# mom-ocean/MOM6

Measured on AMD Instinct MI355X. Metric: simulated-days/wall-sec, higher is better.
Workload: dtype f64

## Files before the change

### mom6_amd/csrc/barotropic.hip

```cpp
#include <algorithm>
#include <type_traits>
#include <vector>
#include <cmath>
#include "mom6x_dev.h"


enum BTW {
  W_q = 0, W_DCor_u, W_DCor_v, W_gtot_E, W_gtot_W, W_gtot_N, W_gtot_S, W_eta, W_eta_PF,
  W_Cor_ref_u, W_Cor_ref_v, W_BT_force_u, W_BT_force_v, W_ubt, W_vbt, W_bt_rem_u, W_bt_rem_v,
  W_uhbt0, W_vhbt0, W_ubt_Cor, W_vbt_Cor, W_uhbt, W_vhbt, W_u_accel_bt, W_v_accel_bt,
  W_eta_src, W_e_anom, W_eta_sum, W_eta_wtd, W_ubt_wtd, W_vbt_wtd, W_eta_pred,
  W_uh0sum, W_vh0sum, W_ubt0, W_vbt0,
  W_f4u, W_f4u_2, W_f4u_3, W_f4u_4, W_f4v, W_f4v_2, W_f4v_3, W_f4v_4,
  W_BTCu,
  W_BTCv = W_BTCu + 10,
  W_BTtmp = W_BTCv + 10,
  W_uhn = W_BTtmp + 12,
  W_vhn,
  W_ubt2, W_vbt2, W_eta_pred2,
  W_COUNT
};

enum BTC { B_FA_EE = 0, B_FA_E0, B_FA_W0, B_FA_WW, B_uBT_WW, B_uBT_EE, B_crvW, B_crvE, B_uh_WW, B_uh_EE };

struct BTState {
  mom6x_barotropic_params P;
  double *frhatu, *frhatv, *IDatu, *IDatv, *ubtav, *vbtav, *eta_cor, *q_D, *D_u_Cor, *D_v_Cor;
  double *work;
  int nstep_last;
  unsigned long long *warn;
  double *warn_info;
  bool la_pending;
  const double *la_pbce;
  double la_underflow;
  bool fr_pending;
  const double *fr_hu, *fr_hv;
};

namespace {

__device__ __forceinline__ double *wp(double *work, const Dm &d, int m) { return work + (size_t)m * d.slab; }

__device__ __forceinline__ double find_uhbt(double u, const double *__restrict__ B, size_t c, size_t slab) {
  if (u == 0.0) return 0.0;
  const double uEE = B[B_uBT_EE * slab + c];
  if (u < uEE) return (u - uEE) * B[B_FA_EE * slab + c] + B[B_uh_EE * slab + c];
  if (u < 0.0) return u * (B[B_FA_E0 * slab + c] + B[B_crvE * slab + c] * (u * u));
  const double uWW = B[B_uBT_WW * slab + c];
  if (u <= uWW) return u * (B[B_FA_W0 * slab + c] + B[B_crvW * slab + c] * (u * u));
  return (u - uWW) * B[B_FA_WW * slab + c] + B[B_uh_WW * slab + c];
}

__global__ void k_bt_init_static(Dm d, const double *__restrict__ G, double Z_to_H, double Mean_SL,
                                 double cor_scale, double H_subroundoff, double *q_D, double *D_u_Cor,
                                 double *D_v_Cor, double *IDatu, double *IDatv) {
  const int i = -1 + blockIdx.x * blockDim.x + threadIdx.x;
  const int j = -1 + blockIdx.y * blockDim.y + threadIdx.y;
  if (i > d.ni - 1 || j > d.nj - 1) return;
  const int st = d.pitch;
  const size_t c = ix2(d, i, j);
  const double *bathyT = gm(G, d, MOM6X_G_bathyT), *areaT = gm(G, d, MOM6X_G_areaT), *mT = gm(G, d, MOM6X_G_mask2dT);
  const double *mCu = gm(G, d, MOM6X_G_mask2dCu), *mCv = gm(G, d, MOM6X_G_mask2dCv), *fBu = gm(G, d, MOM6X_G_CoriolisBu);
  if (j >= 0) {
    D_u_Cor[c] = 0.5 * (dmax(Mean_SL + bathyT[c + 1], 0.0) + dmax(Mean_SL + bathyT[c], 0.0)) * Z_to_H;
    if (mCu[c] > 0.) IDatu[c] = mCu[c] * 2.0 / (Z_to_H * ((bathyT[c + 1] + bathyT[c]) + 2.0 * Mean_SL));
    else IDatu[c] = 0.;
  }
  if (i >= 0) {
    D_v_Cor[c] = 0.5 * (dmax(Mean_SL + bathyT[c + st], 0.0) + dmax(Mean_SL + bathyT[c], 0.0)) * Z_to_H;
    if (mCv[c] > 0.) IDatv[c] = mCv[c] * 2.0 / (Z_to_H * ((bathyT[c + st] + bathyT[c]) + 2.0 * Mean_SL));
    else IDatv[c] = 0.;
  }
  if (mT[c] + mT[c + st] + mT[c + 1] + mT[c + 1 + st] > 0.) {
    q_D[c] = 0.25 * (cor_scale * fBu[c]) * ((areaT[c] + areaT[c + 1 + st]) + (areaT[c + 1] + areaT[c + st])) /
        (Z_to_H * dmax((((areaT[c] * dmax(Mean_SL + bathyT[c], 0.0)) +
                         (areaT[c + 1 + st] * dmax(Mean_SL + bathyT[c + 1 + st], 0.0))) +
                        ((areaT[c + 1] * dmax(Mean_SL + bathyT[c + 1], 0.0)) +
                         (areaT[c + st] * dmax(Mean_SL + bathyT[c + st], 0.0)))), H_subroundoff));
  } else {
    q_D[c] = 0.;
  }
}

// ... 243 lines not shown
    tmp[0 * slab + c] = -1.0e100; tmp[1 * slab + c] = 1.0e100;
    tmp[2 * slab + c] = Dat; tmp[3 * slab + c] = Dat; tmp[4 * slab + c] = Dat; tmp[5 * slab + c] = Dat;
  }
  if (i >= -1) {
    const double H2 = eta ? (bathyT[c + st] * Z_to_H + eta[c + st]) : ((bathyT[c + st] + Z_ref) * Z_to_H);
    double Dat = 0.0;
    if ((H1 > 0.0) && (H2 > 0.0)) Dat = gm(G, d, MOM6X_G_dx_Cv)[c] * (2.0 * H1 * H2) / (H1 + H2);
    tmp[6 * slab + c] = -1.0e100; tmp[7 * slab + c] = 1.0e100;
    tmp[8 * slab + c] = Dat; tmp[9 * slab + c] = Dat; tmp[10 * slab + c] = Dat; tmp[11 * slab + c] = Dat;
  }
}
__global__ void k_face_areas_eta(Dm d, const double *__restrict__ G, double Z_to_H, const double *__restrict__ eta, double *Bu, double *Bv,
                                 int isv, int iev, int jsv, int jev) {
  const int i = isv - 2 + blockIdx.x * blockDim.x + threadIdx.x;
  const int j = jsv - 2 + blockIdx.y * blockDim.y + threadIdx.y;
  if (i > iev + 1 || j > jev + 1) return;
  const int st = d.pitch;
  const size_t c = ix2(d, i, j), slab = (size_t)d.slab;
  const double *bathyT = gm(G, d, MOM6X_G_bathyT);
  const double H1 = bathyT[c] * Z_to_H + eta[c];
  if (j >= jsv - 1) {
    const double H2 = bathyT[c + 1] * Z_to_H + eta[c + 1];
    double Dat = 0.0;
    if ((H1 > 0.0) && (H2 > 0.0)) Dat = gm(G, d, MOM6X_G_dy_Cu)[c] * (2.0 * H1 * H2) / (H1 + H2);
    Bu[B_FA_EE * slab + c] = Dat; Bu[B_FA_E0 * slab + c] = Dat; Bu[B_FA_W0 * slab + c] = Dat; Bu[B_FA_WW * slab + c] = Dat;
  }
  if (i >= isv - 1) {
    const double H2 = bathyT[c + st] * Z_to_H + eta[c + st];
    double Dat = 0.0;
    if ((H1 > 0.0) && (H2 > 0.0)) Dat = gm(G, d, MOM6X_G_dx_Cv)[c] * (2.0 * H1 * H2) / (H1 + H2);
    Bv[B_FA_EE * slab + c] = Dat; Bv[B_FA_E0 * slab + c] = Dat; Bv[B_FA_W0 * slab + c] = Dat; Bv[B_FA_WW * slab + c] = Dat;
  }
}
__global__ void k_btcl(Dm d, const double *__restrict__ tmp, double *Bu, double *Bv, int hs) {
  const int i = -hs - 1 + blockIdx.x * blockDim.x + threadIdx.x;
  const int j = -hs - 1 + blockIdx.y * blockDim.y + threadIdx.y;
  if (i > d.ni - 1 + hs || j > d.nj - 1 + hs) return;
  const size_t c = ix2(d, i, j), slab = (size_t)d.slab;
  const double C1_3 = 1.0 / 3.0;
  for (int dir = 0; dir < 2; dir++) {
    if (dir == 0 && j < -hs) continue;
    if (dir == 1 && i < -hs) continue;
    const double *t = tmp + (size_t)(dir * 6) * slab;
    double *B = dir ? Bv : Bu;
    const double FA_EE = t[2 * slab + c], FA_E0 = t[3 * slab + c], FA_W0 = t[4 * slab + c], FA_WW = t[5 * slab + c];
    const double uBT_EE = 1.0 * t[0 * slab + c], uBT_WW = 1.0 * t[1 * slab + c];
    B[B_FA_EE * slab + c] = FA_EE; B[B_FA_E0 * slab + c] = FA_E0; B[B_FA_W0 * slab + c] = FA_W0; B[B_FA_WW * slab + c] = FA_WW;
    B[B_uBT_EE * slab + c] = uBT_EE; B[B_uBT_WW * slab + c] = uBT_WW;
    B[B_uh_EE * slab + c] = uBT_EE * (C1_3 * (2.0 * FA_E0 + FA_EE));
    B[B_uh_WW * slab + c] = uBT_WW * (C1_3 * (2.0 * FA_W0 + FA_WW));
    double crvW = 0.0, crvE = 0.0;
    if (fabs(uBT_WW) > 0.0) crvW = (C1_3 * (FA_WW - FA_W0)) / (uBT_WW * uBT_WW);
    if (fabs(uBT_EE) > 0.0) crvE = (C1_3 * (FA_EE - FA_E0)) / (uBT_EE * uBT_EE);
    B[B_crvW * slab + c] = crvW; B[B_crvE * slab + c] = crvE;
  }
}

__global__ void k_uhbt0(Dm d, const double *__restrict__ work_c, double *work) {
  const int i = -1 + blockIdx.x * blockDim.x + threadIdx.x;
  const int j = -1 + blockIdx.y * blockDim.y + threadIdx.y;
  if (i > d.ni - 1 || j > d.nj - 1) return;
  const size_t c = ix2(d, i, j), slab = (size_t)d.slab;
  if (j >= 0) work[W_uhbt0 * slab + c] = work_c[W_uh0sum * slab + c] - find_uhbt(work_c[W_ubt0 * slab + c], work_c + W_BTCu * slab, c, slab);
  if (i >= 0) work[W_vhbt0 * slab + c] = work_c[W_vh0sum * slab + c] - find_uhbt(work_c[W_vbt0 * slab + c], work_c + W_BTCv * slab, c, slab);
}

__global__ void k_find_Cor(Dm d, double *work, int Sadourny, int isvf, int ievf, int jsvf, int jevf) {
  const int i = isvf - 1 + blockIdx.x * blockDim.x + threadIdx.x;
  const int j = jsvf - 1 + blockIdx.y * blockDim.y + threadIdx.y;
  if (i > ievf + 1 || j > jevf + 1) return;
  const int st = d.pitch;
  const size_t c = ix2(d, i, j), slab = (size_t)d.slab;
  const double *q = work + W_q * slab, *DCor_u = work + W_DCor_u * slab, *DCor_v = work + W_DCor_v * slab;
  double *f4u = work + W_f4u * slab, *f4v = work + W_f4v * slab;
  if (j <= jevf) {
    if (Sadourny) {
      f4v[0 * slab + c] = 1.0 * DCor_u[c - 1] * q[c - 1];
      f4v[1 * slab + c] = 1.0 * DCor_u[c] * q[c];
      f4v[3 * slab + c] = 1.0 * DCor_u[c + st] * q[c];
      f4v[2 * slab + c] = 1.0 * DCor_u[c - 1 + st] * q[c - 1];
    } else {
      f4v[0 * slab + c] = 1.0 * DCor_u[c - 1] * ((q[c] + q[c - 1 - st]) + q[c - 1]) / 3.0;
      f4v[1 * slab + c] = 1.0 * DCor_u[c] * (q[c] + (q[c - 1] + q[c - st])) / 3.0;
      f4v[3 * slab + c] = 1.0 * DCor_u[c + st] * (q[c] + (q[c - 1] + q[c + st])) / 3.0;
      f4v[2 * slab + c] = 1.0 * DCor_u[c - 1 + st] * ((q[c] + q[c - 1 + st]) + q[c - 1]) / 3.0;
    }
  }
  if (i <= ievf) {
    if (Sadourny) {
      f4u[3 * slab + c] = 1.0 * DCor_v[c + 1] * q[c];
      f4u[2 * slab + c] = 1.0 * DCor_v[c] * q[c];
      f4u[0 * slab + c] = 1.0 * DCor_v[c - st] * q[c - st];
      f4u[1 * slab + c] = 1.0 * DCor_v[c + 1 - st] * q[c - st];
    } else {
      f4u[3 * slab + c] = 1.0 * DCor_v[c + 1] * (q[c] + (q[c + 1] + q[c - st])) / 3.0;
      f4u[2 * slab + c] = 1.0 * DCor_v[c] * (q[c] + (q[c - 1] + q[c - st])) / 3.0;
      f4u[0 * slab + c] = 1.0 * DCor_v[c - st] * ((q[c] + q[c - 1 - st]) + q[c - st]) / 3.0;
      f4u[1 * slab + c] = 1.0 * DCor_v[c + 1 - st] * ((q[c] + q[c + 1 - st]) + q[c - st]) / 3.0;
    }
  }
}

__global__ void k_cor_ref_eta_src(Dm d, const double *__restrict__ G, double *work, double *eta_cor, double Instep,
                                  int bound_BT_corr, double maxCFL_Idt, double dt, double Z_to_H, double Z_ref, double maxvel) {
  const int i = -1 + blockIdx.x * blockDim.x + threadIdx.x;
  const int j = -1 + blockIdx.y * blockDim.y + threadIdx.y;
  if (i > d.ni - 1 || j > d.nj - 1) return;
  const int st = d.pitch;
  const size_t c = ix2(d, i, j), slab = (size_t)d.slab;
  const double *f4u = work + W_f4u * slab, *f4v = work + W_f4v * slab;
  const double *ubt_Cor = work + W_ubt_Cor * slab, *vbt_Cor = work + W_vbt_Cor * slab;
  if (j >= 0)
    work[W_Cor_ref_u * slab + c] = (((f4u[3 * slab + c] * vbt_Cor[c + 1]) + (f4u[0 * slab + c] * vbt_Cor[c - st])) +
                                    ((f4u[2 * slab + c] * vbt_Cor[c]) + (f4u[1 * slab + c] * vbt_Cor[c + 1 - st])));
  if (i >= 0)
    work[W_Cor_ref_v * slab + c] = -1.0 * (((f4v[0 * slab + c] * ubt_Cor[c - 1]) + (f4v[3 * slab + c] * ubt_Cor[c + st])) +
                                           ((f4v[1 * slab + c] * ubt_Cor[c]) + (f4v[2 * slab + c] * ubt_Cor[c - 1 + st])));
  if (i >= 0 && j >= 0) {
    const double mT = gm(G, d, MOM6X_G_mask2dT)[c];
    double ec = eta_cor[c];
    if (bound_BT_corr == 2) {
      const double *bathyT = gm(G, d, MOM6X_G_bathyT), *dy_Cu = gm(G, d, MOM6X_G_dy_Cu), *dx_Cv = gm(G, d, MOM6X_G_dx_Cv);
      auto Dat = [&](size_t a, size_t bb, double len) {
        const double H1 = (bathyT[a] + Z_ref) * Z_to_H, H2 = (bathyT[bb] + Z_ref) * Z_to_H;
        double D = 0.0;
        if ((H1 > 0.0) && (H2 > 0.0)) D = len * (2.0 * H1 * H2) / (H1 + H2);
        return D;
      };
      const double DatuW = Dat(c - 1, c, dy_Cu[c - 1]), DatuE = Dat(c, c + 1, dy_Cu[c]);
      const double DatvN = Dat(c, c + st, dx_Cv[c]), DatvS = Dat(c - st, c, dx_Cv[c - st]);
      const double bound = dt * (gm(G, d, MOM6X_G_IareaT)[c] * 0.1 * maxvel * ((DatuW + DatuE) + (DatvN + DatvS)));
      if (fabs(ec) > bound) ec = copysign(bound, ec);
      eta_cor[c] = ec;
    } else if (bound_BT_corr && mT > 0.0) {
      if (ec > 0.0) {
        const double u_max_cor = gm(G, d, MOM6X_G_dxT)[c] * maxCFL_Idt, v_max_cor = gm(G, d, MOM6X_G_dyT)[c] * maxCFL_Idt;
        const double *Bu = work + W_BTCu * slab, *Bv = work + W_BTCv * slab;
        const double *uhbt0 = work + W_uhbt0 * slab, *vhbt0 = work + W_vhbt0 * slab;
        const double eta_cor_max = dt * (gm(G, d, MOM6X_G_IareaT)[c] *
            (((find_uhbt(u_max_cor, Bu, c, slab) + uhbt0[c]) - (find_uhbt(-u_max_cor, Bu, c - 1, slab) + uhbt0[c - 1])) +
             ((find_uhbt(v_max_cor, Bv, c, slab) + vhbt0[c]) - (find_uhbt(-v_max_cor, Bv, c - st, slab) + vhbt0[c - st]))));
        ec = dmin(ec, dmax(0.0, eta_cor_max));
      } else {
        const double Htot = gm(G, d, MOM6X_G_bathyT)[c] * Z_to_H + work[W_eta * slab + c];
        ec = dmax(ec, -dmax(0.0, Htot));
      }
      eta_cor[c] = ec;
    }
    work[W_eta_src * slab + c] = mT * (Instep * ec);
  }
// ... 24 lines not shown
__global__ void __launch_bounds__(256)
k_bt_pred(Dm d, const double *__restrict__ G, double *work, LoopArgs A, int p_ubt, int p_vbt, int p_pred, int sel) {
  const int i = I_BASE(A.isv - 1) + blockIdx.x * blockDim.x + threadIdx.x;
  const int j = A.jsv - 1 + blockIdx.y * blockDim.y + threadIdx.y;
  if (i < A.isv - 1 || i > A.iev + 1 || j > A.jev + 1) return;
  if (sel) { const bool own = (i >= 0 && i <= d.ni - 1 && j >= 0 && j <= d.nj - 1); if (own != (sel == 1)) return; }
  const int st = d.pitch;
  const size_t c = ix2(d, i, j), slab = (size_t)d.slab;
  double eta_PF_BT;
  if (A.project) {
    eta_PF_BT = work[W_eta * slab + c];
  } else {
    const double *ubt = work + (size_t)p_ubt * slab, *vbt = work + (size_t)p_vbt * slab;
    const double *Bu = work + W_BTCu * slab, *Bv = work + W_BTCv * slab;
    const double *uhbt0 = work + W_uhbt0 * slab, *vhbt0 = work + W_vhbt0 * slab;
    double uW, uE, vS, vN;
    if (A.have_uhn) {
      const double *uhn = work + W_uhn * slab, *vhn = work + W_vhn * slab;
      uW = uhn[c - 1]; uE = uhn[c]; vS = vhn[c - st]; vN = vhn[c];
    } else {
      uW = find_uhbt(ubt[c - 1], Bu, c - 1, slab) + uhbt0[c - 1];
      uE = find_uhbt(ubt[c], Bu, c, slab) + uhbt0[c];
      vS = find_uhbt(vbt[c - st], Bv, c - st, slab) + vhbt0[c - st];
      vN = find_uhbt(vbt[c], Bv, c, slab) + vhbt0[c];
    }
    eta_PF_BT = (work[W_eta * slab + c] + work[W_eta_src * slab + c]) +
                (A.dtbt * gm(G, d, MOM6X_G_IareaT)[c]) * ((uW - uE) + (vS - vN));
    work[(size_t)p_pred * slab + c] = eta_PF_BT;
  }
  if (A.find_etaav && (fabs(A.wt_accel2) > 0.0) && i >= 0 && i <= d.ni - 1 && j >= 0 && j <= d.nj - 1)
    work[W_eta_sum * slab + c] = work[W_eta_sum * slab + c] + A.wt_accel2 * eta_PF_BT;
}

__device__ __forceinline__ void f4u_of(const double *__restrict__ q, const double *__restrict__ DCor_v, size_t c, int st, int Sadourny,
                                       double &f0, double &f1, double &f2, double &f3) {
  if (Sadourny) {
    f3 = 1.0 * DCor_v[c + 1] * q[c];
    f2 = 1.0 * DCor_v[c] * q[c];
    f0 = 1.0 * DCor_v[c - st] * q[c - st];
    f1 = 1.0 * DCor_v[c + 1 - st] * q[c - st];
  } else {
    f3 = 1.0 * DCor_v[c + 1] * (q[c] + (q[c + 1] + q[c - st])) / 3.0;
    f2 = 1.0 * DCor_v[c] * (q[c] + (q[c - 1] + q[c - st])) / 3.0;
    f0 = 1.0 * DCor_v[c - st] * ((q[c] + q[c - 1 - st]) + q[c - st]) / 3.0;
    f1 = 1.0 * DCor_v[c + 1 - st] * ((q[c] + q[c + 1 - st]) + q[c - st]) / 3.0;
  }
}
__device__ __forceinline__ void f4v_of(const double *__restrict__ q, const double *__restrict__ DCor_u, size_t c, int st, int Sadourny,
                                       double &f0, double &f1, double &f2, double &f3) {
  if (Sadourny) {
    f0 = 1.0 * DCor_u[c - 1] * q[c - 1];
    f1 = 1.0 * DCor_u[c] * q[c];
    f3 = 1.0 * DCor_u[c + st] * q[c];
    f2 = 1.0 * DCor_u[c - 1 + st] * q[c - 1];
  } else {
    f0 = 1.0 * DCor_u[c - 1] * ((q[c] + q[c - 1 - st]) + q[c - 1]) / 3.0;
    f1 = 1.0 * DCor_u[c] * (q[c] + (q[c - 1] + q[c - st])) / 3.0;
    f3 = 1.0 * DCor_u[c + st] * (q[c] + (q[c - 1] + q[c + st])) / 3.0;
    f2 = 1.0 * DCor_u[c - 1 + st] * ((q[c] + q[c - 1 + st]) + q[c - 1]) / 3.0;
  }
}

template <int DIR>
__device__ __forceinline__ void bt_face_update(const Dm &d, const double *__restrict__ G, const double *work, const LoopArgs &A, size_t c, int st,
                                               size_t slab, const double *etaB, double vel, double n0, double n1, double n2, double n3,
                                               int bracket_bug, double &newv, double &CorPF) {
  const double *eta_PF = work + W_eta_PF * slab;
  double Cor, PF, f0, f1, f2, f3;
  if (DIR == 0) {
    const double *gE = work + W_gtot_E * slab, *gW = work + W_gtot_W * slab;
    PF = (((etaB[c] - eta_PF[c]) * gE[c]) - ((etaB[c + 1] - eta_PF[c + 1]) * gW[c + 1])) * A.dgeo_de * gm(G, d, MOM6X_G_IdxCu)[c];
    f4u_of(work + W_q * slab, work + W_DCor_v * slab, c, st, A.Sadourny, f0, f1, f2, f3);
    Cor = (((f3 * n0) + (f0 * n1)) + ((f2 * n2) + (f1 * n3))) - work[W_Cor_ref_u * slab + c];
    newv = work[W_bt_rem_u * slab + c] * (vel + A.dtbt * ((work[W_BT_force_u * slab + c] + Cor) + PF));
  } else {
    const double *gN = work + W_gtot_N * slab, *gS = work + W_gtot_S * slab;
    PF = (((etaB[c] - eta_PF[c]) * gN[c]) - ((etaB[c + st] - eta_PF[c + st]) * gS[c + st])) * A.dgeo_de * gm(G, d, MOM6X_G_IdyCv)[c];
    f4v_of(work + W_q * slab, work + W_DCor_u * slab, c, st, A.Sadourny, f0, f1, f2, f3);
    if (bracket_bug) Cor = -1.0 * (((f0 * n0) + (f1 * n1)) + ((f3 * n2) + (f2 * n3))) - work[W_Cor_ref_v * slab + c];
    else Cor = -1.0 * (((f0 * n0) + (f3 * n2)) + ((f1 * n1) + (f2 * n3))) - work[W_Cor_ref_v * slab + c];
    newv = work[W_bt_rem_v * slab + c] * (vel + A.dtbt * ((work[W_BT_force_v * slab + c] + Cor) + PF));
  }
  if (fabs(newv) < A.vel_underflow) newv = 0.0;
  CorPF = Cor + PF;
}

template <int DIR>
__global__ void __launch_bounds__(256)
k_bt_vel(Dm d, const double *__restrict__ G, double *work, double *btav, double *hbtav, LoopArgs A,
         int a0, int a1, int b0, int b1, int bracket_bug) {
  const int i = I_BASE(a0) + blockIdx.x * blockDim.x + threadIdx.x;
  const int j = b0 + blockIdx.y * blockDim.y + threadIdx.y;
  if (i < a0 || i > a1 || j > b1) return;
  const int st = d.pitch;
  const size_t c = ix2(d, i, j), slab = (size_t)d.slab;
// ... 530 lines not shown
  Au.Instep = Instep; Au.RZ_to_H = c->GV.RZ_to_H; Au.vel_underflow = P.vel_underflow; Au.nstep = nstep;
  Au.wt_uv_bug = P.wt_uv_bug; Au.visc_rem_u_uh0 = P.visc_rem_u_uh0; Au.strong_drag = P.strong_drag;
  ColArgs Av = Au;
  Av.visc_rem = visc_rem_v; Av.frhat = s->frhatv; Av.U_Cor = V_Cor; Av.uh0 = vh0; Av.u_uh0 = v_vh0; Av.U_in = V_in;
  Av.bc_accel = bc_accel_v; Av.tau = tauy; Av.tau_bot = tauy_bot; Av.IDat = s->IDatv;
  Av.ubt_Cor = work + W_vbt_Cor * slab; Av.gtot_m = work + W_gtot_N * slab; Av.gtot_p = work + W_gtot_S * slab;
  Av.uh0sum = work + W_vh0sum * slab; Av.ubt0 = work + W_vbt0 * slab; Av.ubt = work + W_vbt * slab;
  Av.BT_force = work + W_BT_force_v * slab; Av.bt_rem = work + W_bt_rem_v * slab;
  if (s->fr_pending) {
    Au.hf = s->fr_hu; Av.hf = s->fr_hv; Au.h_neglect = Av.h_neglect = c->GV.H_subroundoff;
    KLAUNCH(c, "k_bt_col<0>", (k_bt_col<0, true>), grid3(nxa(d.ni + 1, -1), d.nj, 1, b), b, d, c->G, Au);
    KLAUNCH(c, "k_bt_col<1>", (k_bt_col<1, true>), grid3(d.ni, d.nj + 1, 1, b), b, d, c->G, Av);
  } else {
    { const int rcm = bt_frhat_materialize(c); if (rcm) return rcm; }
    KLAUNCH(c, "k_bt_col<0>", (k_bt_col<0, false>), grid3(nxa(d.ni + 1, -1), d.nj, 1, b), b, d, c->G, Au);
    KLAUNCH(c, "k_bt_col<1>", (k_bt_col<1, false>), grid3(d.ni, d.nj + 1, 1, b), b, d, c->G, Av);
  }

  double *tmp = work + W_BTtmp * slab;
  if (BT_cont) KLAUNCH(c, "k_btcont_copy", k_btcont_copy, grid3(d.ni + 1, d.nj + 1, 1, b), b, d, *BT_cont, tmp);
  else KLAUNCH(c, "k_face_areas_as_fits", k_face_areas_as_fits, grid3(d.ni + 3, d.nj + 3, 1, b), b, d, c->G, P.Z_ref, c->GV.Z_to_H, tmp,
               P.nonlinear_continuity ? (const double *)(work + W_eta * slab) : (const double *)nullptr);
  {
    double *f[18]; int stg[18], nks[18];
    for (int m = 0; m < 12; m++) { f[m] = tmp + (size_t)m * slab; stg[m] = (m < 6) ? 1 : 2; nks[m] = 1; }
    double *g[] = { work + W_gtot_E * slab, work + W_gtot_N * slab, work + W_gtot_W * slab, work + W_gtot_S * slab,
                    work + W_ubt_Cor * slab, work + W_vbt_Cor * slab };
    const int gs[] = { 0, 0, 0, 0, 1, 2 };
    for (int m = 0; m < 6; m++) { f[12 + m] = g[m]; stg[12 + m] = gs[m]; nks[12 + m] = 1; }
    halo_wrap(c, f, stg, nks, 18);
  }
  const int hs = 1 + ievf - ie;
  KLAUNCH(c, "k_btcl", k_btcl, grid3(d.ni + 2 * hs + 1, d.nj + 2 * hs + 1, 1, b), b, d, tmp, work + W_BTCu * slab,
                     work + W_BTCv * slab, hs);
  if (add_uh0) KLAUNCH(c, "k_uhbt0", k_uhbt0, grid3(d.ni + 1, d.nj + 1, 1, b), b, d, work, work);

  KLAUNCH(c, "k_find_Cor", k_find_Cor, grid3(ievf - isvf + 3, jevf - jsvf + 3, 1, b), b, d, work, P.Sadourny, isvf, ievf, jsvf, jevf);
  KLAUNCH(c, "k_cor_ref_eta_src", k_cor_ref_eta_src, grid3(d.ni + 1, d.nj + 1, 1, b), b, d, c->G, work, s->eta_cor, Instep,
                     P.bound_BT_corr ? ((BT_cont && P.BT_cont_bounds) ? 1 : 2) : 0, P.maxCFL_BT_cont * Idt, dt, c->GV.Z_to_H, P.Z_ref, P.maxvel);
  {
    std::vector<double *> f = { work + W_eta_PF * slab, work + W_eta_src * slab, work + W_bt_rem_u * slab, work + W_bt_rem_v * slab,
                                work + W_BT_force_u * slab, work + W_BT_force_v * slab };
    std::vector<int> stg = { 0, 0, 1, 2, 1, 2 };
    if (add_uh0) { f.push_back(work + W_uhbt0 * slab); stg.push_back(1); f.push_back(work + W_vhbt0 * slab); stg.push_back(2); }
    f.push_back(work + W_Cor_ref_u * slab); stg.push_back(1); f.push_back(work + W_Cor_ref_v * slab); stg.push_back(2);
    std::vector<int> nks(f.size(), 1);
    halo_wrap(c, f.data(), stg.data(), nks.data(), (int)f.size());
  }

  double dt_filt;
  if (P.dt_bt_filter >= 0.0) dt_filt = 0.5 * fmax(0.0, fmin(P.dt_bt_filter, 2.0 * dt));
  else dt_filt = 0.5 * fmax(0.0, dt * fmin(-P.dt_bt_filter, 2.0));
  const int nfilter = (int)ceil(dt_filt / dtbt);
  const int nt = nstep + nfilter;
  REQUIRE(nt > 0, MOM6X_EINVAL, "btstep: number of barotropic step (nstep+nfilter) is 0");
  std::vector<double> wt_vel(nt + 2, 0.0), wt_eta(nt + 2, 0.0), wt_trans(nt + 2, 0.0), wt_accel(nt + 2, 0.0), wt_accel2(nt + 2, 0.0);
  double sum_wt_vel = 0.0, sum_wt_eta = 0.0, sum_wt_accel = 0.0, sum_wt_trans = 0.0;
  for (int n = 1; n <= nt; n++) {
    if ((n == nstep) || (dt_filt - abs(n - nstep) * dtbt >= 0.0)) { wt_vel[n] = 1.0; wt_eta[n] = 1.0; }
    else if (dtbt + dt_filt - abs(n - nstep) * dtbt > 0.0) { wt_vel[n] = 1.0 + (dt_filt / dtbt) - abs(n - nstep); wt_eta[n] = wt_vel[n]; }
    else { wt_vel[n] = 0.0; wt_eta[n] = 0.0; }
    sum_wt_vel = sum_wt_vel + wt_vel[n]; sum_wt_eta = sum_wt_eta + wt_eta[n];
  }
  for (int n = nt; n >= 1; n--) {
    wt_trans[n] = wt_trans[n + 1] + wt_eta[n];
    wt_accel[n] = wt_accel[n + 1] + wt_vel[n];
    sum_wt_accel = sum_wt_accel + wt_accel[n]; sum_wt_trans = sum_wt_trans + wt_trans[n];
  }
  const double I_sum_wt_vel = 1.0 / sum_wt_vel, I_sum_wt_accel = 1.0 / sum_wt_accel;
  const double I_sum_wt_eta = 1.0 / sum_wt_eta, I_sum_wt_trans = 1.0 / sum_wt_trans;
  for (int n = 1; n <= nt; n++) {
// ... 114 lines not shown
```

### mom6_amd/csrc/halo.hip

```cpp
#include <dlfcn.h>
#include <rccl/rccl.h>
#include <mutex>
#include <vector>
#include "mom6x_dev.h"

#define MAXF 24
struct WrapArgs { double *f[MAXF]; int stg[MAXF]; int nk[MAXF]; int n; int rx; int w, w2; int wf[MAXF]; };
#define PASS_W(A, m) (((A).nk[m] == 1) ? (A).w2 : ((A).wf[m] > 0 ? (A).wf[m] : (A).w))

__host__ __device__ inline void dir_dxdy(int d, int &dx, int &dy) {
  const int DX[8] = { -1, 1, 0, 0, -1, 1, -1, 1 }, DY[8] = { 0, 0, -1, 1, -1, -1, 1, 1 };
  dx = DX[d]; dy = DY[d];
}
__host__ __device__ inline int dir_opp(int d) { const int O[8] = { 1, 0, 3, 2, 7, 6, 5, 4 }; return O[d]; }

__host__ __device__ inline void axis_range(int n, int w, int B, int s, int send, int &a0, int &a1) {
  if (s == 0) { a0 = -B; a1 = n - 1; }
  else if (send) { if (s > 0) { a0 = n - w - B; a1 = n - 1 - B; } else { a0 = 0; a1 = w - 1; } }
  else { if (s > 0) { a0 = n; a1 = n + w - 1; } else { a0 = -w - B; a1 = -1 - B; } }
}

extern "C" int mom6x_halo_region(const mom6x_dims *d, int stagger, int dir, int send, int *i0, int *i1, int *j0, int *j1) {
  if (!d || dir < 0 || dir > 7 || stagger < 0 || stagger > 3) return MOM6X_EINVAL;
  int dx, dy; dir_dxdy(dir, dx, dy);
// ... 26 lines not shown
    axis_range(d.ni, PASS_W(A, m), xB, dx, send, i0, i1);
    axis_range(d.nj, PASS_W(A, m), yB, dy, send, j0, j1);
    const unsigned nx = (unsigned)(i1 - i0 + 1), ny = (unsigned)(j1 - j0 + 1);
    const unsigned per_k = nx * ny, tot = per_k * (unsigned)A.nk[m];
    double *__restrict__ fld = A.f[m];
    for (unsigned t = blockIdx.x * blockDim.x + threadIdx.x; t < tot; t += gridDim.x * blockDim.x) {
      const unsigned k = t / per_k;
      const unsigned r = t - k * per_k;
      const unsigned jj = r / nx, ii = r - jj * nx;
      const size_t x = ix3(d, i0 + (int)ii, j0 + (int)jj, (int)k);
      if (send) buf[off + t] = fld[x];
      else fld[x] = buf[off + t];
    }
    off += tot;
  }
}

static size_t region_count(const mom6x_dims &d, const WrapArgs &A, int dir) {
  int dx, dy; dir_dxdy(dir, dx, dy);
  size_t tot = 0;
  for (int m = 0; m < A.n; m++) {
    const int xB = (A.stg[m] == 1 || A.stg[m] == 3), yB = (A.stg[m] == 2 || A.stg[m] == 3);
    int i0, i1, j0, j1;
    axis_range(d.ni, PASS_W(A, m), xB, dx, 1, i0, i1);
    axis_range(d.nj, PASS_W(A, m), yB, dy, 1, j0, j1);
    tot += (size_t)(i1 - i0 + 1) * (j1 - j0 + 1) * A.nk[m];
  }
  return tot;
}

__global__ void k_wrap_x(Dm d, WrapArgs A) {
  const int jj = blockIdx.x * blockDim.x + threadIdx.x;
  const int hh = threadIdx.y;
  const int k = blockIdx.z;
  const int ni = d.ni;
  for (int m = 0; m < A.n; m++) {
    if (k >= A.nk[m]) continue;
    const int w = PASS_W(A, m);
    const int xB = (A.stg[m] == 1 || A.stg[m] == 3), yB = (A.stg[m] == 2 || A.stg[m] == 3);
    const int j = -yB + jj;
    if (j > d.nj - 1) continue;
    double *p = A.f[m] + (size_t)k * d.slab;
    if (hh < w) {
      const int iw = -w - xB + hh;
      p[ix2(d, iw, j)] = p[ix2(d, iw + ni, j)];
      const int ie = ni + hh;
      p[ix2(d, ie, j)] = p[ix2(d, ie - ni, j)];
    }
  }
}

__global__ void k_wrap_y(Dm d, WrapArgs A) {
  const int ii = blockIdx.x * blockDim.x + threadIdx.x;
  const int hh = threadIdx.y;
  const int k = blockIdx.z;
  const int nj = d.nj;
  for (int m = 0; m < A.n; m++) {
    if (k >= A.nk[m]) continue;
    const int w = PASS_W(A, m);
    const int xB = (A.stg[m] == 1 || A.stg[m] == 3), yB = (A.stg[m] == 2 || A.stg[m] == 3);
    const int i = (A.rx ? -w - xB : -xB) + ii;
    if (i > d.ni - 1 + (A.rx ? w : 0)) continue;
    double *p = A.f[m] + (size_t)k * d.slab;
    if (hh < w) {
      const int js = -w - yB + hh;
      p[ix2(d, i, js)] = p[ix2(d, i, js + nj)];
      const int jn = nj + hh;
      p[ix2(d, i, jn)] = p[ix2(d, i, jn - nj)];
    }
  }
}

struct Nbr8 { int on[8]; };
__global__ void __launch_bounds__(256)
k_halo_poison(Dm d, WrapArgs A, Nbr8 N) {
  const int nrows = d.slab / d.pitch;
  const unsigned per_k = (unsigned)d.pitch * (unsigned)nrows;
  const double bad = __longlong_as_double(0x7ff8000000000000LL);
  for (int m = 0; m < A.n; m++) {
    const int w = PASS_W(A, m);
    if (w >= d.halo) continue;
    const int xB = (A.stg[m] == 1 || A.stg[m] == 3), yB = (A.stg[m] == 2 || A.stg[m] == 3);
    const unsigned tot = per_k * (unsigned)A.nk[m];
    for (unsigned t = blockIdx.x * blockDim.x + threadIdx.x; t < tot; t += gridDim.x * blockDim.x) {
      const unsigned k = t / per_k, r = t - k * per_k;
      const int j = (int)(r / (unsigned)d.pitch) - d.joff, i = (int)(r % (unsigned)d.pitch) - d.ioff;
      if (i < -d.halo - xB || i > d.ni - 1 + d.halo || j < -d.halo - yB || j > d.nj - 1 + d.halo) continue;
      const int sx = (i < -xB) ? -1 : ((i > d.ni - 1) ? 1 : 0), sy = (j < -yB) ? -1 : ((j > d.nj - 1) ? 1 : 0);
      if (sx == 0 && sy == 0) continue;
      int dir = -1;
      for (int q = 0; q < 8; q++) { int dx, dy; dir_dxdy(q, dx, dy); if (dx == sx && dy == sy) dir = q; }
      if (!N.on[dir]) continue;
      const int dist_x = (sx < 0) ? (-xB - i) : ((sx > 0) ? i - (d.ni - 1) : 0), dist_y = (sy < 0) ? (-yB - j) : ((sy > 0) ? j - (d.nj - 1) : 0);
      if (dist_x > w || dist_y > w) A.f[m][(size_t)k * d.slab + r] = bad;
    }
  }
}
static bool poison_halo() { static const bool on = [] { const char *e = getenv("MOM6X_POISON_HALO"); return e && *e && *e != '0'; }(); return on; }

struct NcclApi {
  ncclResult_t (*GetUniqueId)(ncclUniqueId *);
  ncclResult_t (*CommInitRank)(ncclComm_t *, int, ncclUniqueId, int);
  ncclResult_t (*CommDestroy)(ncclComm_t);
// ... 243 lines not shown
    hipLaunchKernelGGL(k_halo_poison, dim3(512), dim3(256), 0, st, d, A, N);
  }
  return MOM6X_OK;
}

static WrapArgs wrap_args(const mom6x_ctx *c, double *const *fields, const int *staggers, const int *nks, int base, int n,
                          const PassWidth &pw) {
  WrapArgs A;
  A.n = n; A.rx = c->dims.reentrant_x;
  A.w = (pw.w > 0 && pw.w < c->dims.halo) ? pw.w : c->dims.halo; A.w2 = c->dims.halo;
  for (int q = 0; q < n; q++) {
    A.f[q] = fields[base + q]; A.stg[q] = staggers[base + q]; A.nk[q] = nks[base + q];
    A.wf[q] = (base + q < pw.nwf && pw.wf[base + q] > 0 && pw.wf[base + q] < A.w) ? pw.wf[base + q] : 0;
  }
  return A;
}

void halo_wrap(mom6x_ctx *c, double *const *fields, const int *staggers, const int *nks, int n, PassWidth pw) {
  const Dm d = c->d;
  Comm *m = c->comm;
  if (c->pass_pending) halo_complete(c);
  if (!m && !c->dims.reentrant_x && !c->dims.reentrant_y) return;
  for (int base = 0; base < n; base += MAXF) {
    const WrapArgs A = wrap_args(c, fields, staggers, nks, base, (n - base < MAXF) ? (n - base) : MAXF, pw);
    int nkmax = 1;
    for (int q = 0; q < A.n; q++) { if (A.nk[q] > nkmax) nkmax = A.nk[q]; }
    if (m) {
      if (exchange(c, m, A, c->stream) != MOM6X_OK) c->halo_error = true;
      continue;
    }
    const dim3 b(64, d.halo, 1);
    if (c->dims.reentrant_x) {
      const int rows = d.nj + 2 * d.halo + 1;
      KLAUNCH(c, "k_wrap_x", k_wrap_x, dim3((rows + 63) / 64, 1, nkmax), b, d, A);
    }
    if (c->dims.reentrant_y) {
      const int cols = d.ni + 2 * d.halo + 1;
      KLAUNCH(c, "k_wrap_y", k_wrap_y, dim3((cols + 63) / 64, 1, nkmax), b, d, A);
    }
    if (poison_halo()) {
      Nbr8 N;
      for (int dir = 0; dir < 8; dir++) {
        int dx, dy; dir_dxdy(dir, dx, dy);
        N.on[dir] = (dx == 0 || c->dims.reentrant_x) && (dy == 0 || c->dims.reentrant_y);
      }
      hipLaunchKernelGGL(k_halo_poison, dim3(512), dim3(256), 0, c->stream, d, A, N);
    }
  }
}

void halo_start(mom6x_ctx *c, double *const *fields, const int *staggers, const int *nks, int n, PassWidth pw) {
  Comm *m = c->comm;
  if (!m || !m->comm || n > MAXF) { halo_wrap(c, fields, staggers, nks, n, pw); return; }
  if (c->pass_pending) halo_complete(c);
  if (!c->ev_ready) {
    if (hipEventCreateWithFlags(&c->ev_ready, hipEventDisableTiming) != hipSuccess ||
        hipEventCreateWithFlags(&c->ev_done, hipEventDisableTiming) != hipSuccess) { c->halo_error = true; return; }
  }
  const WrapArgs A = wrap_args(c, fields, staggers, nks, 0, n, pw);
  if (hipEventRecord(c->ev_ready, c->stream) != hipSuccess || hipStreamWaitEvent(c->halo_stream, c->ev_ready, 0) != hipSuccess ||
      exchange(c, m, A, c->halo_stream) != MOM6X_OK || hipEventRecord(c->ev_done, c->halo_stream) != hipSuccess) {
    c->halo_error = true;
    return;
  }
  c->pass_pending = true;
}
bool halo_start_packed(mom6x_ctx *c, double *const *fields, const int *staggers, const int *nks, int n, PassWidth pw) {
  Comm *m = c->comm;
  if (!m || !m->comm || n > MAXF) { halo_wrap(c, fields, staggers, nks, n, pw); return false; }
  if (c->pass_pending) halo_complete(c);
  if (!c->ev_ready) {
// ... 64 lines not shown
```

Measured before the change: 0.1950.

## Fuse barotropic setup kernels and parallelize halo wraps across fields

Folds the uhbt0 computation into k_btcl, using the freshly computed fit coefficients held in registers. It also drops the f4u/f4v work arrays by recomputing the Coriolis stencil coefficients inline in k_cor_ref_eta_src. The halo wrap kernels now put fields on grid.y instead of looping over them serially, and they wrap source indices modulo the domain size. Together this removes two kernel launches and several slab-sized memory round trips per barotropic setup, at the cost of some redundant arithmetic and a change in periodic-wrap source indexing.

```diff
diff --git a/mom6_amd/csrc/barotropic.hip b/mom6_amd/csrc/barotropic.hip
--- a/mom6_amd/csrc/barotropic.hip
+++ b/mom6_amd/csrc/barotropic.hip
@@ -11,7 +11,6 @@
   W_uhbt0, W_vhbt0, W_ubt_Cor, W_vbt_Cor, W_uhbt, W_vhbt, W_u_accel_bt, W_v_accel_bt,
   W_eta_src, W_e_anom, W_eta_sum, W_eta_wtd, W_ubt_wtd, W_vbt_wtd, W_eta_pred,
   W_uh0sum, W_vh0sum, W_ubt0, W_vbt0,
-  W_f4u, W_f4u_2, W_f4u_3, W_f4u_4, W_f4v, W_f4v_2, W_f4v_3, W_f4v_4,
   W_BTCu,
   W_BTCv = W_BTCu + 10,
   W_BTtmp = W_BTCv + 10,
@@ -49,6 +48,15 @@
   const double uWW = B[B_uBT_WW * slab + c];
   if (u <= uWW) return u * (B[B_FA_W0 * slab + c] + B[B_crvW * slab + c] * (u * u));
   return (u - uWW) * B[B_FA_WW * slab + c] + B[B_uh_WW * slab + c];
+}
+
+__device__ __forceinline__ double find_uhbt_fit(double u, double FA_EE, double FA_E0, double FA_W0, double FA_WW, double uBT_WW, double uBT_EE,
+                                                double crvW, double crvE, double uh_WW, double uh_EE) {
+  if (u == 0.0) return 0.0;
+  if (u < uBT_EE) return (u - uBT_EE) * FA_EE + uh_EE;
+  if (u < 0.0) return u * (FA_E0 + crvE * (u * u));
+  if (u <= uBT_WW) return u * (FA_W0 + crvW * (u * u));
+  return (u - uBT_WW) * FA_WW + uh_WW;
 }
 
 __global__ void k_bt_init_static(Dm d, const double *__restrict__ G, double Z_to_H, double Mean_SL,
@@ -358,12 +366,13 @@
     Bv[B_FA_EE * slab + c] = Dat; Bv[B_FA_E0 * slab + c] = Dat; Bv[B_FA_W0 * slab + c] = Dat; Bv[B_FA_WW * slab + c] = Dat;
   }
 }
-__global__ void k_btcl(Dm d, const double *__restrict__ tmp, double *Bu, double *Bv, int hs) {
+__global__ void k_btcl(Dm d, const double *__restrict__ tmp, double *Bu, double *Bv, int hs, double *work, int add_uh0) {
   const int i = -hs - 1 + blockIdx.x * blockDim.x + threadIdx.x;
   const int j = -hs - 1 + blockIdx.y * blockDim.y + threadIdx.y;
   if (i > d.ni - 1 + hs || j > d.nj - 1 + hs) return;
   const size_t c = ix2(d, i, j), slab = (size_t)d.slab;
   const double C1_3 = 1.0 / 3.0;
+  const bool uh0_here = add_uh0 && i >= -1 && i <= d.ni - 1 && j >= -1 && j <= d.nj - 1;
   for (int dir = 0; dir < 2; dir++) {
     if (dir == 0 && j < -hs) continue;
     if (dir == 1 && i < -hs) continue;
@@ -373,75 +382,66 @@
     const double uBT_EE = 1.0 * t[0 * slab + c], uBT_WW = 1.0 * t[1 * slab + c];
     B[B_FA_EE * slab + c] = FA_EE; B[B_FA_E0 * slab + c] = FA_E0; B[B_FA_W0 * slab + c] = FA_W0; B[B_FA_WW * slab + c] = FA_WW;
     B[B_uBT_EE * slab + c] = uBT_EE; B[B_uBT_WW * slab + c] = uBT_WW;
-    B[B_uh_EE * slab + c] = uBT_EE * (C1_3 * (2.0 * FA_E0 + FA_EE));
-    B[B_uh_WW * slab + c] = uBT_WW * (C1_3 * (2.0 * FA_W0 + FA_WW));
+    const double uh_EE = uBT_EE * (C1_3 * (2.0 * FA_E0 + FA_EE)), uh_WW = uBT_WW * (C1_3 * (2.0 * FA_W0 + FA_WW));
+    B[B_uh_EE * slab + c] = uh_EE;
+    B[B_uh_WW * slab + c] = uh_WW;
     double crvW = 0.0, crvE = 0.0;
     if (fabs(uBT_WW) > 0.0) crvW = (C1_3 * (FA_WW - FA_W0)) / (uBT_WW * uBT_WW);
     if (fabs(uBT_EE) > 0.0) crvE = (C1_3 * (FA_EE - FA_E0)) / (uBT_EE * uBT_EE);
     B[B_crvW * slab + c] = crvW; B[B_crvE * slab + c] = crvE;
-  }
-}
-
-__global__ void k_uhbt0(Dm d, const double *__restrict__ work_c, double *work) {
-  const int i = -1 + blockIdx.x * blockDim.x + threadIdx.x;
-  const int j = -1 + blockIdx.y * blockDim.y + threadIdx.y;
-  if (i > d.ni - 1 || j > d.nj - 1) return;
-  const size_t c = ix2(d, i, j), slab = (size_t)d.slab;
-  if (j >= 0) work[W_uhbt0 * slab + c] = work_c[W_uh0sum * slab + c] - find_uhbt(work_c[W_ubt0 * slab + c], work_c + W_BTCu * slab, c, slab);
-  if (i >= 0) work[W_vhbt0 * slab + c] = work_c[W_vh0sum * slab + c] - find_uhbt(work_c[W_vbt0 * slab + c], work_c + W_BTCv * slab, c, slab);
-}
-
-__global__ void k_find_Cor(Dm d, double *work, int Sadourny, int isvf, int ievf, int jsvf, int jevf) {
-  const int i = isvf - 1 + blockIdx.x * blockDim.x + threadIdx.x;
-  const int j = jsvf - 1 + blockIdx.y * blockDim.y + threadIdx.y;
-  if (i > ievf + 1 || j > jevf + 1) return;
-  const int st = d.pitch;
-  const size_t c = ix2(d, i, j), slab = (size_t)d.slab;
-  const double *q = work + W_q * slab, *DCor_u = work + W_DCor_u * slab, *DCor_v = work + W_DCor_v * slab;
-  double *f4u = work + W_f4u * slab, *f4v = work + W_f4v * slab;
-  if (j <= jevf) {
-    if (Sadourny) {
-      f4v[0 * slab + c] = 1.0 * DCor_u[c - 1] * q[c - 1];
-      f4v[1 * slab + c] = 1.0 * DCor_u[c] * q[c];
-      f4v[3 * slab + c] = 1.0 * DCor_u[c + st] * q[c];
-      f4v[2 * slab + c] = 1.0 * DCor_u[c - 1 + st] * q[c - 1];
-    } else {
-      f4v[0 * slab + c] = 1.0 * DCor_u[c - 1] * ((q[c] + q[c - 1 - st]) + q[c - 1]) / 3.0;
-      f4v[1 * slab + c] = 1.0 * DCor_u[c] * (q[c] + (q[c - 1] + q[c - st])) / 3.0;
-      f4v[3 * slab + c] = 1.0 * DCor_u[c + st] * (q[c] + (q[c - 1] + q[c + st])) / 3.0;
-      f4v[2 * slab + c] = 1.0 * DCor_u[c - 1 + st] * ((q[c] + q[c - 1 + st]) + q[c - 1]) / 3.0;
-    }
-  }
-  if (i <= ievf) {
-    if (Sadourny) {
-      f4u[3 * slab + c] = 1.0 * DCor_v[c + 1] * q[c];
-      f4u[2 * slab + c] = 1.0 * DCor_v[c] * q[c];
-      f4u[0 * slab + c] = 1.0 * DCor_v[c - st] * q[c - st];
-      f4u[1 * slab + c] = 1.0 * DCor_v[c + 1 - st] * q[c - st];
-    } else {
-      f4u[3 * slab + c] = 1.0 * DCor_v[c + 1] * (q[c] + (q[c + 1] + q[c - st])) / 3.0;
-      f4u[2 * slab + c] = 1.0 * DCor_v[c] * (q[c] + (q[c - 1] + q[c - st])) / 3.0;
-      f4u[0 * slab + c] = 1.0 * DCor_v[c - st] * ((q[c] + q[c - 1 - st]) + q[c - st]) / 3.0;
-      f4u[1 * slab + c] = 1.0 * DCor_v[c + 1 - st] * ((q[c] + q[c + 1 - st]) + q[c - st]) / 3.0;
-    }
-  }
-}
-
-__global__ void k_cor_ref_eta_src(Dm d, const double *__restrict__ G, double *work, double *eta_cor, double Instep,
+    if (uh0_here && (dir ? (i >= 0) : (j >= 0)))
+      work[(dir ? W_vhbt0 : W_uhbt0) * slab + c] = work[(dir ? W_vh0sum : W_uh0sum) * slab + c] -
+          find_uhbt_fit(work[(dir ? W_vbt0 : W_ubt0) * slab + c], FA_EE, FA_E0, FA_W0, FA_WW, uBT_WW, uBT_EE, crvW, crvE, uh_WW, uh_EE);
+  }
+}
+
+__device__ __forceinline__ void f4u_of(const double *__restrict__ q, const double *__restrict__ DCor_v, size_t c, int st, int Sadourny,
+                                       double &f0, double &f1, double &f2, double &f3) {
+  if (Sadourny) {
+    f3 = 1.0 * DCor_v[c + 1] * q[c];
+    f2 = 1.0 * DCor_v[c] * q[c];
+    f0 = 1.0 * DCor_v[c - st] * q[c - st];
+    f1 = 1.0 * DCor_v[c + 1 - st] * q[c - st];
+  } else {
+    f3 = 1.0 * DCor_v[c + 1] * (q[c] + (q[c + 1] + q[c - st])) / 3.0;
+    f2 = 1.0 * DCor_v[c] * (q[c] + (q[c - 1] + q[c - st])) / 3.0;
+    f0 = 1.0 * DCor_v[c - st] * ((q[c] + q[c - 1 - st]) + q[c - st]) / 3.0;
+    f1 = 1.0 * DCor_v[c + 1 - st] * ((q[c] + q[c + 1 - st]) + q[c - st]) / 3.0;
+  }
+}
+__device__ __forceinline__ void f4v_of(const double *__restrict__ q, const double *__restrict__ DCor_u, size_t c, int st, int Sadourny,
+                                       double &f0, double &f1, double &f2, double &f3) {
+  if (Sadourny) {
+    f0 = 1.0 * DCor_u[c - 1] * q[c - 1];
+    f1 = 1.0 * DCor_u[c] * q[c];
+    f3 = 1.0 * DCor_u[c + st] * q[c];
+    f2 = 1.0 * DCor_u[c - 1 + st] * q[c - 1];
+  } else {
+    f0 = 1.0 * DCor_u[c - 1] * ((q[c] + q[c - 1 - st]) + q[c - 1]) / 3.0;
+    f1 = 1.0 * DCor_u[c] * (q[c] + (q[c - 1] + q[c - st])) / 3.0;
+    f3 = 1.0 * DCor_u[c + st] * (q[c] + (q[c - 1] + q[c + st])) / 3.0;
+    f2 = 1.0 * DCor_u[c - 1 + st] * ((q[c] + q[c - 1 + st]) + q[c - 1]) / 3.0;
+  }
+}
+
+__global__ void k_cor_ref_eta_src(Dm d, const double *__restrict__ G, double *work, double *eta_cor, double Instep, int Sadourny,
                                   int bound_BT_corr, double maxCFL_Idt, double dt, double Z_to_H, double Z_ref, double maxvel) {
   const int i = -1 + blockIdx.x * blockDim.x + threadIdx.x;
   const int j = -1 + blockIdx.y * blockDim.y + threadIdx.y;
   if (i > d.ni - 1 || j > d.nj - 1) return;
   const int st = d.pitch;
   const size_t c = ix2(d, i, j), slab = (size_t)d.slab;
-  const double *f4u = work + W_f4u * slab, *f4v = work + W_f4v * slab;
+  const double *q = work + W_q * slab;
   const double *ubt_Cor = work + W_ubt_Cor * slab, *vbt_Cor = work + W_vbt_Cor * slab;
-  if (j >= 0)
-    work[W_Cor_ref_u * slab + c] = (((f4u[3 * slab + c] * vbt_Cor[c + 1]) + (f4u[0 * slab + c] * vbt_Cor[c - st])) +
-                                    ((f4u[2 * slab + c] * vbt_Cor[c]) + (f4u[1 * slab + c] * vbt_Cor[c + 1 - st])));
-  if (i >= 0)
-    work[W_Cor_ref_v * slab + c] = -1.0 * (((f4v[0 * slab + c] * ubt_Cor[c - 1]) + (f4v[3 * slab + c] * ubt_Cor[c + st])) +
-                                           ((f4v[1 * slab + c] * ubt_Cor[c]) + (f4v[2 * slab + c] * ubt_Cor[c - 1 + st])));
+  double f0, f1, f2, f3;
+  if (j >= 0) {
+    f4u_of(q, work + W_DCor_v * slab, c, st, Sadourny, f0, f1, f2, f3);
+    work[W_Cor_ref_u * slab + c] = (((f3 * vbt_Cor[c + 1]) + (f0 * vbt_Cor[c - st])) + ((f2 * vbt_Cor[c]) + (f1 * vbt_Cor[c + 1 - st])));
+  }
+  if (i >= 0) {
+    f4v_of(q, work + W_DCor_u * slab, c, st, Sadourny, f0, f1, f2, f3);
+    work[W_Cor_ref_v * slab + c] = -1.0 * (((f0 * ubt_Cor[c - 1]) + (f3 * ubt_Cor[c + st])) + ((f1 * ubt_Cor[c]) + (f2 * ubt_Cor[c - 1 + st])));
+  }
   if (i >= 0 && j >= 0) {
     const double mT = gm(G, d, MOM6X_G_mask2dT)[c];
     double ec = eta_cor[c];
@@ -532,35 +532,6 @@
     work[W_eta_sum * slab + c] = work[W_eta_sum * slab + c] + A.wt_accel2 * eta_PF_BT;
 }
 
-__device__ __forceinline__ void f4u_of(const double *__restrict__ q, const double *__restrict__ DCor_v, size_t c, int st, int Sadourny,
-                                       double &f0, double &f1, double &f2, double &f3) {
-  if (Sadourny) {
-    f3 = 1.0 * DCor_v[c + 1] * q[c];
-    f2 = 1.0 * DCor_v[c] * q[c];
-    f0 = 1.0 * DCor_v[c - st] * q[c - st];
-    f1 = 1.0 * DCor_v[c + 1 - st] * q[c - st];
-  } else {
-    f3 = 1.0 * DCor_v[c + 1] * (q[c] + (q[c + 1] + q[c - st])) / 3.0;
-    f2 = 1.0 * DCor_v[c] * (q[c] + (q[c - 1] + q[c - st])) / 3.0;
-    f0 = 1.0 * DCor_v[c - st] * ((q[c] + q[c - 1 - st]) + q[c - st]) / 3.0;
-    f1 = 1.0 * DCor_v[c + 1 - st] * ((q[c] + q[c + 1 - st]) + q[c - st]) / 3.0;
-  }
-}
-__device__ __forceinline__ void f4v_of(const double *__restrict__ q, const double *__restrict__ DCor_u, size_t c, int st, int Sadourny,
-                                       double &f0, double &f1, double &f2, double &f3) {
-  if (Sadourny) {
-    f0 = 1.0 * DCor_u[c - 1] * q[c - 1];
-    f1 = 1.0 * DCor_u[c] * q[c];
-    f3 = 1.0 * DCor_u[c + st] * q[c];
-    f2 = 1.0 * DCor_u[c - 1 + st] * q[c - 1];
-  } else {
-    f0 = 1.0 * DCor_u[c - 1] * ((q[c] + q[c - 1 - st]) + q[c - 1]) / 3.0;
-    f1 = 1.0 * DCor_u[c] * (q[c] + (q[c - 1] + q[c - st])) / 3.0;
-    f3 = 1.0 * DCor_u[c + st] * (q[c] + (q[c - 1] + q[c + st])) / 3.0;
-    f2 = 1.0 * DCor_u[c - 1 + st] * ((q[c] + q[c - 1 + st]) + q[c - 1]) / 3.0;
-  }
-}
-
 template <int DIR>
 __device__ __forceinline__ void bt_face_update(const Dm &d, const double *__restrict__ G, const double *work, const LoopArgs &A, size_t c, int st,
                                                size_t slab, const double *etaB, double vel, double n0, double n1, double n2, double n3,
@@ -1157,11 +1128,8 @@
   }
   const int hs = 1 + ievf - ie;
   KLAUNCH(c, "k_btcl", k_btcl, grid3(d.ni + 2 * hs + 1, d.nj + 2 * hs + 1, 1, b), b, d, tmp, work + W_BTCu * slab,
-                     work + W_BTCv * slab, hs);
-  if (add_uh0) KLAUNCH(c, "k_uhbt0", k_uhbt0, grid3(d.ni + 1, d.nj + 1, 1, b), b, d, work, work);
-
-  KLAUNCH(c, "k_find_Cor", k_find_Cor, grid3(ievf - isvf + 3, jevf - jsvf + 3, 1, b), b, d, work, P.Sadourny, isvf, ievf, jsvf, jevf);
-  KLAUNCH(c, "k_cor_ref_eta_src", k_cor_ref_eta_src, grid3(d.ni + 1, d.nj + 1, 1, b), b, d, c->G, work, s->eta_cor, Instep,
+                     work + W_BTCv * slab, hs, work, add_uh0 ? 1 : 0);
+  KLAUNCH(c, "k_cor_ref_eta_src", k_cor_ref_eta_src, grid3(d.ni + 1, d.nj + 1, 1, b), b, d, c->G, work, s->eta_cor, Instep, P.Sadourny,
                      P.bound_BT_corr ? ((BT_cont && P.BT_cont_bounds) ? 1 : 2) : 0, P.maxCFL_BT_cont * Idt, dt, c->GV.Z_to_H, P.Z_ref, P.maxvel);
   {
     std::vector<double *> f = { work + W_eta_PF * slab, work + W_eta_src * slab, work + W_bt_rem_u * slab, work + W_bt_rem_v * slab,
diff --git a/mom6_amd/csrc/halo.hip b/mom6_amd/csrc/halo.hip
--- a/mom6_amd/csrc/halo.hip
+++ b/mom6_amd/csrc/halo.hip
@@ -82,43 +82,43 @@
 __global__ void k_wrap_x(Dm d, WrapArgs A) {
   const int jj = blockIdx.x * blockDim.x + threadIdx.x;
   const int hh = threadIdx.y;
+  const int m = blockIdx.y;
   const int k = blockIdx.z;
   const int ni = d.ni;
-  for (int m = 0; m < A.n; m++) {
-    if (k >= A.nk[m]) continue;
-    const int w = PASS_W(A, m);
-    const int xB = (A.stg[m] == 1 || A.stg[m] == 3), yB = (A.stg[m] == 2 || A.stg[m] == 3);
-    const int j = -yB + jj;
-    if (j > d.nj - 1) continue;
-    double *p = A.f[m] + (size_t)k * d.slab;
-    if (hh < w) {
-      const int iw = -w - xB + hh;
-      p[ix2(d, iw, j)] = p[ix2(d, iw + ni, j)];
-      const int ie = ni + hh;
-      p[ix2(d, ie, j)] = p[ix2(d, ie - ni, j)];
-    }
-  }
+  if (k >= A.nk[m]) return;
+  const int w = PASS_W(A, m);
+  const int xB = (A.stg[m] == 1 || A.stg[m] == 3), yB = (A.stg[m] == 2 || A.stg[m] == 3);
+  const int j = -yB + jj;
+  if (j > d.nj - 1 || hh >= w) return;
+  double *p = A.f[m] + (size_t)k * d.slab;
+  const int iw = -w - xB + hh, ie = ni + hh;
+  int sw = iw + ni, se = ie - ni;
+  while (sw < -xB) sw += ni;
+  while (se > ni - 1) se -= ni;
+  const double fromE = p[ix2(d, sw, j)], fromW = p[ix2(d, se, j)];
+  p[ix2(d, iw, j)] = fromE;
+  p[ix2(d, ie, j)] = fromW;
 }
 
 __global__ void k_wrap_y(Dm d, WrapArgs A) {
   const int ii = blockIdx.x * blockDim.x + threadIdx.x;
   const int hh = threadIdx.y;
+  const int m = blockIdx.y;
   const int k = blockIdx.z;
   const int nj = d.nj;
-  for (int m = 0; m < A.n; m++) {
-    if (k >= A.nk[m]) continue;
-    const int w = PASS_W(A, m);
-    const int xB = (A.stg[m] == 1 || A.stg[m] == 3), yB = (A.stg[m] == 2 || A.stg[m] == 3);
-    const int i = (A.rx ? -w - xB : -xB) + ii;
-    if (i > d.ni - 1 + (A.rx ? w : 0)) continue;
-    double *p = A.f[m] + (size_t)k * d.slab;
-    if (hh < w) {
-      const int js = -w - yB + hh;
-      p[ix2(d, i, js)] = p[ix2(d, i, js + nj)];
-      const int jn = nj + hh;
-      p[ix2(d, i, jn)] = p[ix2(d, i, jn - nj)];
-    }
-  }
+  if (k >= A.nk[m]) return;
+  const int w = PASS_W(A, m);
+  const int xB = (A.stg[m] == 1 || A.stg[m] == 3), yB = (A.stg[m] == 2 || A.stg[m] == 3);
+  const int i = (A.rx ? -w - xB : -xB) + ii;
+  if (i > d.ni - 1 + (A.rx ? w : 0) || hh >= w) return;
+  double *p = A.f[m] + (size_t)k * d.slab;
+  const int js = -w - yB + hh, jn = nj + hh;
+  int ss = js + nj, sn = jn - nj;
+  while (ss < -yB) ss += nj;
+  while (sn > nj - 1) sn -= nj;
+  const double fromN = p[ix2(d, i, ss)], fromS = p[ix2(d, i, sn)];
+  p[ix2(d, i, js)] = fromN;
+  p[ix2(d, i, jn)] = fromS;
 }
 
 struct Nbr8 { int on[8]; };
@@ -428,11 +428,11 @@
     const dim3 b(64, d.halo, 1);
     if (c->dims.reentrant_x) {
       const int rows = d.nj + 2 * d.halo + 1;
-      KLAUNCH(c, "k_wrap_x", k_wrap_x, dim3((rows + 63) / 64, 1, nkmax), b, d, A);
+      KLAUNCH(c, "k_wrap_x", k_wrap_x, dim3((rows + 63) / 64, A.n, nkmax), b, d, A);
     }
     if (c->dims.reentrant_y) {
       const int cols = d.ni + 2 * d.halo + 1;
-      KLAUNCH(c, "k_wrap_y", k_wrap_y, dim3((cols + 63) / 64, 1, nkmax), b, d, A);
+      KLAUNCH(c, "k_wrap_y", k_wrap_y, dim3((cols + 63) / 64, A.n, nkmax), b, d, A);
     }
     if (poison_halo()) {
       Nbr8 N;
```

Result: no change. 0.1965 (median of 6 runs) (+0.8%).
